# dkogan/horizonator

Hardware: AMD Instinct MI355X
Metric: panorama Mpix/s (360deg, 16k-wide, 7x7 SRTM3 tiles) (higher is better)
Workload: dtype f32

## Files before the change

horizonator_amd/_lib.py:

```python
import ctypes as C
import os

_HERE = os.path.dirname(os.path.abspath(__file__))
LIB_PATH = os.environ.get("HORIZONATOR_AMD_LIB") or os.path.join(_HERE, "libhorizonator.so")
DEMGEN_PATH = os.path.join(_HERE, "libhzdemgen.so")
SELFTEST_PATH = os.path.join(_HERE, "libhorizonator_selftest.so")

MAX_NDEMS_IJ = 4


class DemContext(C.Structure):
    _fields_ = [
        ("dems", (C.c_void_p * MAX_NDEMS_IJ) * MAX_NDEMS_IJ),
        ("mmap_sizes", (C.c_size_t * MAX_NDEMS_IJ) * MAX_NDEMS_IJ),
        ("mmap_fd", (C.c_int * MAX_NDEMS_IJ) * MAX_NDEMS_IJ),
        ("origin_dem_lon_lat", C.c_int * 2),
        ("origin_dem_cellij", C.c_int * 2),
        ("Ndems_ij", C.c_int * 2),
        ("radius_cells", C.c_int),
        ("cells_per_deg", C.c_int),
    ]


class _Offscreen(C.Structure):
# ... 2 lines not shown
        ("frameBufID", C.c_uint32),
        ("renderBufID", C.c_uint32),
        ("depthBufID", C.c_uint32),
        ("width", C.c_int),
        ("height", C.c_int),
    ]


class Context(C.Structure):
    _fields_ = (
        [("Ntriangles", C.c_int), ("render_texture", C.c_bool), ("use_glut", C.c_bool),
         ("glut_window", C.c_int)]
        + [(name, C.c_int32) for name in (
            "uniform_aspect", "uniform_az_deg0", "uniform_az_deg1",
            "uniform_viewer_cell_i", "uniform_viewer_cell_j", "uniform_viewer_z",
            "uniform_viewer_lat", "uniform_cos_viewer_lat",
            "uniform_texturemap_lon0", "uniform_texturemap_lon1",
            "uniform_texturemap_dlat0", "uniform_texturemap_dlat1", "uniform_texturemap_dlat2",
            "uniform_znear", "uniform_zfar", "uniform_znear_color", "uniform_zfar_color")]
        + [("program", C.c_uint32), ("viewer_lat", C.c_float), ("viewer_lon", C.c_float),
           ("dems", DemContext), ("offscreen", _Offscreen)]
    )


class View(C.Structure):
    _fields_ = [(n, C.c_float) for n in (
        "viewer_cell_i", "viewer_cell_j", "viewer_z", "cos_viewer_lat", "deg_per_cell",
        "az_deg0", "az_deg1", "aspect", "znear", "zfar", "znear_color", "zfar_color")]


class Options(C.Structure):
    _fields_ = [(n, C.c_int) for n in (
        "serial", "rounds", "near_cells", "coarse_depth", "tiles", "tile_list", "adapt", "adapt_hi", "pretest_march",
        "worklists", "fast_math", "resolve_clears", "queue_capacity", "host_dense", "host_sectors", "host_times", "vertex_cache")]


class Times(C.Structure):
    _fields_ = [(n, C.c_float) for n in ("clear_ms", "raster_ms", "big_ms", "resolve_ms", "total_ms", "near_ms")]


class Window(C.Structure):
    _fields_ = [("cells_per_deg", C.c_int), ("radius_cells", C.c_int),
                ("origin_tile", C.c_int * 2), ("origin_cell", C.c_int * 2)]


class TexParams(C.Structure):
    _fields_ = [(n, C.c_float) for n in ("viewer_lat_rad", "origin_cell_lon_deg", "origin_cell_lat_deg",
                                         "lon0", "lon1", "dlat0", "dlat1", "dlat2")] + \
               [(n, C.c_int32) for n in ("ntiles_x", "ntiles_y", "lowest_x", "lowest_y", "tex_w", "tex_h")]


RASTER_AUTO, RASTER_SCATTER, RASTER_MARCH = 0, 1, 2

_lib = None
_selftest = None


def load():
    global _lib
    if _lib is None:
        _lib = _open(LIB_PATH, selftest=os.path.basename(LIB_PATH) == os.path.basename(SELFTEST_PATH))
    return _lib


def load_selftest():
    global _selftest
    if _selftest is None:
# ... 79 lines not shown
    sig("hz_hip_set_options", i, vp, P(Options))
    sig("hz_hip_set_texture", i, vp, P(TexParams), vp)
    sig("hz_hip_pack", i, vp, vp)
    sig("hz_hip_resolve_packed", i, vp, P(View), vp, vp, i, i, i, vp, vp)
    sig("hz_hip_pack_sparse", i, vp, vp, i)
    sig("hz_hip_resolve_sparse", i, vp, P(View), vp, vp, i, i, i, vp, vp)
    sig("hz_hip_resolve_sparse_strips", i, vp, P(View), vp, i, vp, i, vp, vp, vp, vp)
    sig("hz_hip_draw", i, vp, P(View))
    sig("hz_hip_resolve", i, vp, P(View), vp, vp, vp, vp, vp)
    sig("hz_hip_resolve_to_host", i, vp, P(View), vp, vp, vp, vp, vp)
    sig("hz_hip_render_to_host", i, vp, P(View), vp, vp, vp, vp, vp)
    sig("hz_hip_host_begin", i, vp, P(View), vp, vp, vp, vp, vp)
    sig("hz_hip_host_end", i, vp)
    sig("hz_hip_host_prepare", i, vp, i, i, i, i, vp)
    sig("hz_hip_read_depth", i, vp, i, i, P(C.c_uint32))
    sig("hz_hip_link_cells", i, vp, P(View), vp, vp, vp, vp, d, d, d, i, i, i, i, vp, vp)
    sig("hz_hip_poi_visibility", i, vp, P(View), vp, i, vp, i, vp, vp, vp)
    sig("hz_hip_sync", i, vp)
    sig("hz_hip_last_times", i, vp, P(Times))
    sig("hz_hip_stream", vp, vp)
    sig("hz_hip_wait_outputs", i, vp, vp)
    sig("hz_hip_wait_for", i, vp, vp)
    sig("horizonator_amd_stream_waits_for_outputs", b, ctxp, vp)
    sig("horizonator_amd_waits_for_stream", b, ctxp, vp)
    sig("hz_hip_last_plan", i, vp, vp)
    sig("hz_hip_last_queue_counts", i, vp, vp)
    sig("hz_hip_last_error", C.c_char_p)
    if selftest:
        sig("hz_hip_check_fastmath", i, i, i, C.c_uint64, C.c_uint64, P(C.c_uint64), vp)
        sig("hz_hip_check_exactness", i, i, i, C.c_uint64, C.c_uint64, i, i, i, i, P(C.c_uint64))
        sig("hz_hip_debug_bigqueue", i, vp, i, vp, i, vp)
        sig("hz_hip_debug_wave_timing", i, vp, P(View), vp, C.c_size_t, vp)
        sig("hz_hip_debug_worklist", C.c_long, i, i, i, P(View), i, i, i, vp, C.c_size_t)
    return lib


DECLARED_SYMBOLS = [
    "horizonator_init", "horizonator_deinit", "horizonator_resized", "horizonator_pan_zoom",
    "horizonator_move", "horizonator_set_zextents", "horizonator_redraw", "horizonator_pick",
    "horizonator_render_offscreen", "horizonator_x_from_az", "horizonator_project",
    "horizonator_unproject",
    "horizonator_dem_init", "horizonator_dem_deinit", "horizonator_dem_sample",
    "horizonator_dem_bounds_latlon_deg",
    "horizonator_amd_get_window", "horizonator_amd_init_from_mosaic",
    "horizonator_amd_render", "horizonator_amd_render_device", "horizonator_amd_render_batch",
    "horizonator_amd_render_packed", "horizonator_amd_resolve_packed",
    "horizonator_amd_resolve_packed_strips", "horizonator_amd_render_sparse",
    "horizonator_amd_resolve_sparse_strips",
    "horizonator_amd_sync", "horizonator_amd_stream_waits_for_outputs", "horizonator_amd_waits_for_stream", "horizonator_amd_texture_layout", "horizonator_amd_set_texture",
    "horizonator_amd_set_sector", "horizonator_amd_set_raster", "horizonator_amd_set_profiling",
    "horizonator_amd_get_options", "horizonator_amd_set_options", "horizonator_amd_render_begin", "horizonator_amd_render_end",
    "horizonator_amd_last_times", "horizonator_amd_get_view", "horizonator_amd_device",
    "horizonator_amd_get_mosaic", "horizonator_amd_link_cells_size", "horizonator_amd_link_cells",
    "horizonator_amd_poi_visibility", "horizonator_amd_build_id",
    "hz_hip_device_count", "hz_hip_create", "hz_hip_destroy", "hz_hip_upload_mosaic",
    "hz_hip_download_mosaic", "hz_hip_ingest_tiles", "hz_hip_set_sector", "hz_hip_set_raster",
    "hz_hip_set_profiling", "hz_hip_get_options", "hz_hip_set_options", "hz_hip_set_texture", "hz_hip_pack", "hz_hip_resolve_packed", "hz_hip_pack_sparse", "hz_hip_resolve_sparse", "hz_hip_resolve_sparse_strips", "hz_hip_draw", "hz_hip_resolve", "hz_hip_resolve_to_host", "hz_hip_render_to_host", "hz_hip_host_begin", "hz_hip_host_end", "hz_hip_host_prepare",
    "hz_hip_read_depth", "hz_hip_link_cells", "hz_hip_poi_visibility", "hz_hip_sync", "hz_hip_last_times", "hz_hip_stream", "hz_hip_wait_outputs", "hz_hip_wait_for", "hz_hip_last_plan", "hz_hip_last_queue_counts", "hz_hip_last_error",
]
SELFTEST_SYMBOLS = ["hz_hip_check_fastmath", "hz_hip_check_exactness", "hz_hip_debug_bigqueue", "hz_hip_debug_wave_timing",
                    "hz_hip_debug_worklist"]


def load_demgen():
    if not os.path.exists(DEMGEN_PATH):
        raise ImportError(f"{DEMGEN_PATH} is missing: build it with `make -C horizonator_amd/csrc`")
    lib = C.CDLL(DEMGEN_PATH)
    lib.hz_demgen_write_region.restype = C.c_int
    lib.hz_demgen_write_region.argtypes = [C.c_char_p] + [C.c_int] * 6
    lib.hz_demgen_write_tile.restype = C.c_int
    lib.hz_demgen_write_tile.argtypes = [C.c_char_p] + [C.c_int] * 4
    lib.hz_demgen_tile_values.restype = None
    lib.hz_demgen_tile_values.argtypes = [C.c_void_p] + [C.c_int] * 4
    return lib
```

horizonator_amd/csrc/hz_context.cpp:

```cpp
#include "hz_dev.h"

#include <time.h>

thread_local char hz_g_last_error[512];
extern "C" const char* hz_hip_last_error(void) { return g_last_error; }


static int env_int(const char* name, int dflt) { const char* e = getenv(name); return e ? atoi(e) : dflt; }
static hz_options_t default_options(void)
{
    hz_options_t o;
    o.serial         = 0;
    o.rounds         = 0;
    o.near_cells     = -1;
    o.coarse_depth   = -1;
    o.tiles          = -1;
    o.tile_list      = 0;
    o.adapt          = 1;
    o.adapt_hi       = -1;
    o.pretest_march  = -1;
    o.worklists      = 1;
    o.fast_math      = 1;
    o.resolve_clears = 1;
    o.queue_capacity = 0;
    o.host_dense     = 0;
    o.host_sectors   = 0;
    o.host_times     = 0;
    o.vertex_cache   = 1;
    return o;
}
hz_options_t hz_options_from_env(void)
{
    hz_options_t o = default_options();
    o.serial         = env_int("HZ_SERIAL", o.serial) != 0;
    if(getenv("HZ_TWO_PASS")) o.rounds = env_int("HZ_TWO_PASS", 0) != 0 ? 2 : 1;
    o.near_cells     = env_int("HZ_NEAR_CELLS", o.near_cells);
    if(getenv("HZ_HIZ")) o.coarse_depth = env_int("HZ_HIZ", 0) != 0;
    o.tiles          = env_int("HZ_TILES", o.tiles);
    o.tile_list      = env_int("HZ_TILE_LIST", o.tile_list);
    o.adapt          = env_int("HZ_ADAPT", o.adapt);
    o.adapt_hi       = env_int("HZ_ADAPT_HI", o.adapt_hi);
    if(getenv("HZ_PRETEST_MARCH")) o.pretest_march = env_int("HZ_PRETEST_MARCH", 0) != 0;
    o.worklists      = env_int("HZ_NO_WORKLIST", 0) == 0;
    o.fast_math      = env_int("HZ_NO_FAST_MATH", 0) == 0;
    o.resolve_clears = env_int("HZ_RESOLVE_CLEARS", o.resolve_clears) != 0;
    o.queue_capacity = env_int("HZ_QUEUE_CAPACITY", o.queue_capacity);
    o.host_dense     = env_int("HZ_HOST_DENSE", o.host_dense) != 0;
    o.host_sectors   = env_int("HZ_HOST_SECTORS", o.host_sectors);
    o.host_times     = env_int("HZ_HOST_TIMES", o.host_times) != 0;
    o.vertex_cache   = env_int("HZ_VERTEX_CACHE", o.vertex_cache) != 0;
    return o;
}
#ifdef HZ_EXPERIMENTS
static hz_experiments_t experiments_from_env(void)
{
    hz_experiments_t e = { env_int("HZ_MARCH_DEBUG", 0), env_int("HZ_EXP_FB_MARCH", 0), env_int("HZ_EXP_FB_BIG", 0) };
    return e;
}
#endif
extern "C" int hz_hip_device_count(void)
{
    int n = 0;
    if(hipGetDeviceCount(&n) != hipSuccess) return 0;
    return n;
}

hipError_t hz_sync_all(hz_dev_t* d)
{
    hipError_t rc = hipSuccess;
    hipStream_t all[4] = { d->stream, d->nstream, d->qstream, d->rstream };
    for(int k=0; k<4; k++)
        if(all[k]) { const hipError_t e = hipStreamSynchronize(all[k]); if(e != hipSuccess) rc = e; }
    return rc;
}

extern "C" void hz_hip_destroy(hz_dev_t* d)
{
    if(!d) return;
    hz_device_guard device_guard_(d->device);
    (void)hz_sync_all(d);
    (void)hipFree(d->d_mosaic);
    for(int i=0; i<HZ_NFB; i++) { (void)hipFree(d->d_fbs[i]); (void)hipFree(d->d_touched[i]); }
    for(int i=0; i<2*HZ_NFB; i++)
// ... 329 lines not shown
```

horizonator_amd/csrc/hz_dev.h:

```cpp
#pragma once

#include <hip/hip_runtime_api.h>

#include <math.h>
#include <stdio.h>
#include <stdlib.h>
#include <string.h>
#include <time.h>

#include <vector>

#include "hz_hip.h"
#include "hz_types.h"
#include "hz_launch.h"


extern thread_local char hz_g_last_error[512];
#define g_last_error hz_g_last_error

#define HZ_CHECK(call)                                                        \
    do {                                                                      \
        hipError_t e_ = (call);                                               \
        if(e_ != hipSuccess)                                                  \
        {                                                                     \
// ... 2 lines not shown
            fprintf(stderr, "hz_hip: %s\n", g_last_error);                    \
            return -1;                                                        \
        }                                                                     \
    } while(0)

struct hz_device_guard
{
    int prev, dev; bool ok;
    explicit hz_device_guard(int device) : prev(-1), dev(device), ok(true)
    {
        if(hipGetDevice(&prev) != hipSuccess) prev = -1;
        if(prev != dev)
        {
            const hipError_t e = hipSetDevice(dev);
            if(e != hipSuccess)
            {
                ok = false;
                snprintf(g_last_error, sizeof(g_last_error), "hipSetDevice(%d) -> %s", dev, hipGetErrorString(e));
                fprintf(stderr, "hz_hip: %s\n", g_last_error);
            }
        }
    }
    ~hz_device_guard() { if(ok && prev >= 0 && prev != dev) (void)hipSetDevice(prev); }
};
#define HZ_ON_DEVICE(d) hz_device_guard device_guard_((d)->device); if(!device_guard_.ok) return -1

#ifdef HZ_EXPERIMENTS
struct hz_experiments_t { int march_debug, exp_fb_march, exp_fb_big; };
#endif

struct hz_listkey_t
{
    hz_view_t view; int col0, col1, two_pass, near_x0, near_x1, near_j0, near_j1, far_rows;
};
#define HZ_NLISTS 2
struct hz_worklists_t
{
    uint32_t*    d_items[HZ_NLISTS];
    uint32_t*    h_items[HZ_NLISTS][2];
    size_t       cap[HZ_NLISTS];
    unsigned int n[HZ_NLISTS];
    hipEvent_t   ev_copied[HZ_NLISTS][2];
    int          turn[HZ_NLISTS];
    int          valid;
    unsigned int last_used;
    hz_listkey_t key;
};
#define HZ_LIST_CACHE 8

struct hz_dev
{
    int device;
    hz_options_t env;
#ifdef HZ_EXPERIMENTS
    hz_experiments_t exp;
#endif
    int N, W, H;
    int col0, col1;
    int raster;
    int profiling;
    hz_worklists_t list_cache[HZ_LIST_CACHE];
    hz_worklists_t* lists;
    unsigned int lists_clock;
    std::vector<uint32_t>* list_scratch;
    std::vector<uint32_t>* list_scratch2;
    struct { unsigned long long* d_cycles; size_t capacity; unsigned int grid_x, grid_y; } wave_timing;
// ... 53 lines not shown

    hipEvent_t ev[10];
    int        have_times;
    hz_times_t times;
};

#define HZ_NEAR_PX            20.0f
#define HZ_TWO_ROUNDS_MIN_PIX 6.0e6
#define HZ_TILES_MIN_PX       35.0f
#define HZ_HIZ_MIN_PX         25.0f



struct hz_stopwatch
{
    bool on; timespec t0;
    explicit hz_stopwatch(const char* var) : on(getenv(var) && atoi(getenv(var)) != 0) { clock_gettime(CLOCK_MONOTONIC, &t0); }
    void lap(const char* what)
    {
        if(!on) return;
        timespec t1; clock_gettime(CLOCK_MONOTONIC, &t1);
        fprintf(stderr, "hz_hip init: %-34s %8.2f ms\n", what, 1e3*(double)(t1.tv_sec - t0.tv_sec) + 1e-6*(double)(t1.tv_nsec - t0.tv_nsec));
        t0 = t1;
    }
};


hz_options_t hz_options_from_env(void);
mr_queue_t   hz_queue_set(const hz_dev_t* d, int k);
int          hz_tile_bins(hz_dev_t* d, int set);
hipError_t   hz_sync_all(hz_dev_t* d);
hz_params_t  hz_make_params(const hz_dev_t* d, const hz_view_t* v);
int          hz_plan_rounds(const hz_dev_t* d, const hz_view_t* view, hz_params_t& p);
mr_zones_t   hz_make_zones(const hz_params_t& p, bool near_first);
bool         hz_azimuths_of_columns(const hz_params_t& p, double* a0, double* a1);
void         hz_list_items(const hz_params_t& p, const mr_zones_t& zn, double a0, double a1, std::vector<uint32_t>& out, bool every_strip = false);
void         hz_list_rounds(const hz_params_t& p, const mr_zones_t& zn, double a0, double a1, bool one_round,
                            std::vector<uint32_t>* first, std::vector<uint32_t>& second, bool every_strip = false);
int          hz_draw_impl(hz_dev_t* d, const hz_view_t* view);
int          hz_fb_refill(hz_dev_t* d);
int          hz_fb_mark_consumed(hz_dev_t* d);
int          hz_upload_tanel(hz_dev_t* d, const float* tanel);
int          hz_rstream_after_draw(hz_dev_t* d);
int          hz_resolve_impl(hz_dev_t* d, const hz_view_t* view, const float* tanel,
                             unsigned char* bgr, float* ranges, int32_t* index, uint32_t* z24, int nbands, hipEvent_t* ev_band, int* band_rows);
void         hz_hostpath_destroy(hz_dev_t* d);
int          hz_gpu_numa_node(const hz_dev_t* d);
void         hz_hostpath_landing(hz_dev_t* d, unsigned char** pinned, size_t* bytes);
```

horizonator_amd/csrc/hz_draw.cpp:

```cpp
#include "hz_dev.h"
#include "hz_fast.h"

static int upload_list(hz_dev_t* d, int which, hipStream_t st, const std::vector<uint32_t>& items)
{
    hz_worklists_t& wl = *d->lists;
    const size_t n = items.size();
    if(n > wl.cap[which])
    {
        HZ_CHECK(hz_sync_all(d));
        (void)hipFree(wl.d_items[which]); wl.d_items[which] = NULL;
        for(int t=0; t<2; t++) { if(wl.h_items[which][t]) (void)hipHostFree(wl.h_items[which][t]); wl.h_items[which][t] = NULL; }
        wl.cap[which] = 0;
        const size_t cap = n + n/4 + 1024;
        hipError_t e = hipMalloc(&wl.d_items[which], cap*sizeof(uint32_t));
        for(int t=0; t<2 && e == hipSuccess; t++) e = hipHostMalloc((void**)&wl.h_items[which][t], cap*sizeof(uint32_t), hipHostMallocDefault);
        if(e != hipSuccess)
        {
            (void)hipFree(wl.d_items[which]); wl.d_items[which] = NULL;
            for(int t=0; t<2; t++) { if(wl.h_items[which][t]) (void)hipHostFree(wl.h_items[which][t]); wl.h_items[which][t] = NULL; }
            HZ_CHECK(e);
        }
        wl.cap[which] = cap;
    }
    const int t = wl.turn[which]; wl.turn[which] ^= 1;
// ... 192 lines not shown
                d->adapt.items_short = items;
                const double hi = d->env.adapt_hi >= 0 ? (double)d->env.adapt_hi : 500000.0*((double)(d->col1 - d->col0)*(double)d->H/64.0e6);
                if(!d->adapt.tried_long && (double)items > hi) d->adapt.long_reach = 1;
            }
            else
            {
                d->adapt.tried_long = 1;
                if(!(d->adapt.items_short && (unsigned long long)items*10ull < (unsigned long long)d->adapt.items_short*7ull)) d->adapt.long_reach = 0;
            }
        }
    (void)hipGetLastError();
    if(next_framebuffer(d, p) != 0) return -1;
    const int next = d->fbi;
    if(d->raster != HZ_RASTER_SCATTER && vertex_cache(d, p) != 0) return -1;

    const mr_queue_t q = hz_queue_set(d, next);
    bool by_tile_first = d->env.tiles > 0 && d->raster != HZ_RASTER_SCATTER;
    bool near_beside_far = false;
    bool waited_near = false;
    bool use_hiz = false;
    bool zoomed_view = false;

    if(d->raster == HZ_RASTER_SCATTER)
    {
        HZ_CHECK(hipStreamWaitEvent(d->stream, d->ev_free[next], 0));
        if(prof) { HZ_CHECK(hipEventRecord(d->ev[7], d->stream)); HZ_CHECK(hipEventRecord(d->ev[6], d->stream)); HZ_CHECK(hipEventRecord(d->ev[9], d->stream)); }
        dim3 grid((p.N-1 + SC_CX-1)/SC_CX, (p.N-1 + SC_CY-1)/SC_CY);
        hzk_scatter(grid, dim3(SC_THREADS), d->stream, (const int16_t*)d->d_mosaic, d->d_fb, q, p);
        HZ_CHECK(hipGetLastError());
    }
    else
    {
        const bool two_pass = hz_plan_rounds(d, view, p) == 2;
        const mr_zones_t zn = hz_make_zones(p, two_pass);
        double a0 = 0, a1 = 0;
        const bool listed = d->env.worklists && hz_azimuths_of_columns(p, &a0, &a1) && zn.total < (1 << (32 - MR_ITEM_SX_BITS))
                            && (p.N-1 + MR_COLS-1)/MR_COLS <= (1 << MR_ITEM_SX_BITS);
        p.cull_strips = (p.col0 > 0 || p.col1 < p.W || listed) ? 1 : 0;
        bool fresh_lists = false;
        if(listed)
        {
            hz_listkey_t key;
            memset(&key, 0, sizeof(key));
            key.view = *view; key.col0 = p.col0; key.col1 = p.col1; key.two_pass = two_pass ? 1 : 0;
            key.near_x0 = p.near_x0; key.near_x1 = p.near_x1; key.near_j0 = p.near_j0; key.near_j1 = p.near_j1; key.far_rows = zn.rows[0] | (zn.rows[1] << 8);
            hz_worklists_t* hit = NULL; hz_worklists_t* lru = &d->list_cache[0];
            for(int c=0; c<HZ_LIST_CACHE; c++)
            {
                hz_worklists_t* e = &d->list_cache[c];
                if(e->valid && memcmp(&key, &e->key, sizeof(key)) == 0) { hit = e; break; }
                if((!e->valid && lru->valid) || (e->valid == lru->valid && e->last_used < lru->last_used)) lru = e;
            }
            fresh_lists = hit == NULL;
            d->lists = hit ? hit : lru;
            d->lists->last_used = ++d->lists_clock;
            if(fresh_lists) { d->lists->valid = 0; d->lists->key = key; }
        }
        if(two_pass)
        {
            p.inline_max = HZ_INLINE_MAX_PIX;
            const mr_queue_t qn = hz_queue_set(d, HZ_NFB + next);
            HZ_CHECK(hipStreamWaitEvent(d->nstream, d->ev_free[next], 0));
            {
                const float ppr = p.halfW * p.u.az_ndc_per_rad;
                const float reach = 0.5f*(float)(p.near_j1 - p.near_j0);
                zoomed_view = reach > 0.f && ppr/reach >= HZ_HIZ_MIN_PX;
                const float cells_to_zfar = view->zfar / (p.u.deg_per_cell * 111194.9f);
                p.qshards_log2 = (zoomed_view || cells_to_zfar <= 0.25f*ppr) ? HZ_QSHARDS_LOG2 : 0;
            }
            hz_params_t p1 = p;
            p1.pass = 1; p1.early_z = 0;
            if(fresh_lists)
            {
                hz_list_rounds(p1, zn, a0, a1, false, d->list_scratch, *d->list_scratch2);
                if(upload_list(d, 0, d->nstream, *d->list_scratch) != 0) return -1;
            }
            if(prof) HZ_CHECK(hipEventRecord(d->ev[7], d->nstream));
            if(launch_march(d, d->nstream, qn, zn, p1, listed ? d->lists->d_items[0] : NULL, d->lists->n[0]) != 0) return -1;
// ... 93 lines not shown
```

horizonator_amd/csrc/hz_k_march.h:

```cpp
#pragma once


#define MR_CAP    128
#define MR_RSLOTS 4
#define MR_FIELDS 6

struct mr_lds_t
{
    uint32_t rows[MR_RSLOTS][MR_FIELDS][64];
    uint32_t ids[MR_CAP];
    uint32_t clip[64];
    uint32_t nclip;
};

__device__ static inline void mr_clip_flush(mr_lds_t& L, const mr_queue_t& q, int lane)
{
    const unsigned int nclip = (unsigned int)__builtin_amdgcn_readfirstlane((int)L.nclip);
    if(!nclip) return;
    uint32_t base = 0;
    if(lane == 0) base = atomicAdd(&q.counters[4], nclip);
    base = (uint32_t)__builtin_amdgcn_readfirstlane((int)base);
    if((unsigned int)lane < nclip)
    {
        const uint32_t at = base + (uint32_t)lane;
// ... 376 lines not shown
    }
    if(dbg) { const uint32_t tot = (uint32_t)__builtin_amdgcn_readlane((int)mr_scan(npix, lane), 63); dbg[4] += tot; }
    mr_distribute(r, npix, lane, fb, p);
}

#ifdef MR_WAVES_PER_EU
#define MR_OCCUPANCY __attribute__((amdgpu_waves_per_eu(MR_WAVES_PER_EU, MR_WAVES_PER_EU)))
#elif defined(MR_VGPRS)
#define MR_OCCUPANCY __attribute__((amdgpu_num_vgpr(MR_VGPRS)))
#else
#define MR_OCCUPANCY
#endif
template<bool COUNTERS, bool HIZ, bool VCACHE, bool SHARDS>
__global__ __launch_bounds__(64) MR_OCCUPANCY
void k_march(const int16_t* __restrict__ mosaic, unsigned long long* __restrict__ fb,
             mr_queue_t q, mr_zones_t zn, hz_params_t p)
{
    __shared__ mr_lds_t L;
    const unsigned long long t_start = COUNTERS ? __builtin_amdgcn_s_memtime() : 0ull;
    unsigned int dbgv[6] = {0,0,0,0,0,0};
    unsigned int* dbg = COUNTERS ? dbgv : nullptr;

    const int lane = threadIdx.x;
    int sx, seg;
    if(p.worklist)
    {
        const uint32_t item = p.worklist[blockIdx.x];
        sx = (int)(item & ((1u << MR_ITEM_SX_BITS) - 1u)); seg = (int)(item >> MR_ITEM_SX_BITS);
    }
    else { sx = (int)blockIdx.x + (p.pass == 1 ? p.near_x0 : 0); seg = (int)blockIdx.y; }
    const int i0   = sx*MR_COLS;
    const int i    = i0 + lane;
    int jbeg, jend;
    mr_segment_rows(zn, seg, &jbeg, &jend);
    if(p.pass)
    {
        const bool near = sx >= p.near_x0 && sx <= p.near_x1 && jbeg < p.near_j1 && jend > p.near_j0;
        if((p.pass == 1) != near) return;
    }
    const bool has_vertex = i < p.N;
    const bool has_cell   = lane < MR_COLS && i < p.N-1;
    const int  ic = has_vertex ? i : p.N-1;

    if(p.cull_strips)
    {
        const int ia = i0, ib = min(i0 + MR_COLS, p.N-1);
        const bool viewer_inside = p.u.viewer_cell_i >= (float)(ia-1) && p.u.viewer_cell_i <= (float)(ib+1) &&
                                   p.u.viewer_cell_j >= (float)(jbeg-1) && p.u.viewer_cell_j <= (float)(jend+1);
        if(!viewer_inside)
        {
            const hz_vertex_t v = hz_transform_en(&p.u, hz_east(&p.u, (float)((lane & 1) ? ib : ia)),
                                                  hz_north(&p.u, (float)((lane & 2) ? jend : jbeg)), 0.f);
            float xlo = 2.f, xhi = -2.f;
            #pragma unroll
            for(int c=0; c<4; c++)
            {
                const float xc = __builtin_bit_cast(float, __builtin_amdgcn_readlane(__builtin_bit_cast(int, v.x), c));
                xlo = hz_min(xlo, xc); xhi = hz_max(xhi, xc);
            }
            if(xhi - xlo <= 1.0f)
            {
                const float flo = (xlo*p.halfW + p.halfW) - 2.5f, fhi = (xhi*p.halfW + p.halfW) + 1.5f;
                if(fhi < (float)p.col0 || flo > (float)p.col1) return;
            }
        }
    }

// ... 162 lines not shown
```

horizonator_amd/csrc/hz_plan.cpp:

```cpp
#include "hz_dev.h"
#include "hz_fast.h"

mr_zones_t hz_make_zones(const hz_params_t& p, bool near_first)
{
    const float ppr = p.halfW * p.u.az_ndc_per_rad;
    const int   ncr = p.N-1;
    const float vj  = p.u.viewer_cell_j;
    const int r2  = (int)(ppr/16.f) + 1;
    const int r4  = (int)(ppr/4.f) + 1;
    const int r16 = (int)(ppr/1.f) + 1;
    auto clampi = [&](float x) { int v = (int)floorf(x); if(v < 0) v = 0; if(v > ncr) v = ncr; return v; };
    mr_zones_t z;
    z.row0[0] = 0;
    z.row0[1] = clampi(vj - (float)r16);
    z.row0[2] = clampi(vj - (float)r4);
    z.row0[3] = clampi(vj - (float)r2);
    z.row0[4] = clampi(vj + (float)r2 + 1.f);
    z.row0[5] = clampi(vj + (float)r4 + 1.f);
    z.row0[6] = clampi(vj + (float)r16 + 1.f);
    z.row0[7] = ncr;
    int far_rows = 64*p.SW/p.W;
    if(far_rows < 16) far_rows = 16;
    if(far_rows > 32) far_rows = 32;
    const int z16 = 6*p.SW < p.W ? 8 : 16;
    const float cells_to_zfar = sqrtf(p.far_dd)/(p.u.deg_per_cell*111194.9f);
    const int z4 = cells_to_zfar <= 0.25f*ppr ? 2 : 4;
    int rows[MR_NZONES] = { far_rows, z16, z4, 2, z4, z16, far_rows };
    if(p.SW == p.W)
    {
        long waves = 0;
        for(int k=0; k<MR_NZONES; k++) waves += (z.row0[k+1] - z.row0[k] + rows[k]-1)/rows[k];
        waves *= (p.N-1 + MR_COLS-1)/MR_COLS;
        if(waves < 32768) { rows[0] = rows[6] = rows[0] < 16 ? rows[0] : 16; rows[1] = rows[5] = rows[1] < 8 ? rows[1] : 8; rows[2] = rows[4] = 2; }
    }
    const int order_far_first [MR_NZONES] = { 0, 6, 1, 5, 2, 4, 3 };
    const int order_near_first[MR_NZONES] = { 3, 2, 4, 1, 5, 0, 6 };
    z.near_first = near_first ? 1 : 0;
    const int* order = near_first ? order_near_first : order_far_first;
    int seg = 0;
    for(int o=0; o<MR_NZONES; o++)
    {
        const int k = order[o];
        z.rows[k] = rows[k];
        z.seg0[k] = seg;
        const int n = z.row0[k+1] - z.row0[k];
        z.nseg[k] = (n + rows[k]-1)/rows[k];
        seg += z.nseg[k];
    }
    z.total = seg;
    return z;
}

hz_params_t hz_make_params(const hz_dev_t* d, const hz_view_t* v)
{
    hz_params_t p;
    memset(&p, 0, sizeof(p));
    p.u.viewer_cell_i  = v->viewer_cell_i;
    p.u.viewer_cell_j  = v->viewer_cell_j;
    p.u.viewer_z       = v->viewer_z;
    p.u.cos_viewer_lat = v->cos_viewer_lat;
    p.u.deg_per_cell   = v->deg_per_cell;
    p.u.aspect         = v->aspect;
    p.u.znear          = v->znear;
    p.u.zfar           = v->zfar;
    p.u.znear_color    = v->znear_color;
    p.u.zfar_color     = v->zfar_color;
// ... 85 lines not shown
    }
    if(!any) return false;
    double i_lo = lo/m_per_cell_e + (double)p.u.viewer_cell_i - 2.0, i_hi = hi/m_per_cell_e + (double)p.u.viewer_cell_i + 2.0;
    if(!(i_lo > -1e9)) i_lo = -1e9;
    if(!(i_hi <  1e9)) i_hi =  1e9;
    int a = (int)ceil(i_lo/(double)MR_COLS) - 1, b = (int)floor(i_hi/(double)MR_COLS);
    if(a < 0) a = 0;
    if(b > nsx-1) b = nsx-1;
    if(a > b) return false;
    *x0 = a; *x1 = b;
    return true;
}

bool hz_azimuths_of_columns(const hz_params_t& p, double* a0, double* a1)
{
    const double k = (double)p.u.az_ndc_per_rad, c = (double)p.u.az_center, hw = (double)p.halfW;
    const double lo = c + (((double)p.col0 - 4.0)/hw - 1.0)/k, hi = c + (((double)p.col1 + 4.0)/hw - 1.0)/k;
    if(!(hi - lo < 2.0*M_PI - 1e-3) || !(hi > lo)) return false;
    *a0 = lo; *a1 = hi;
    return true;
}

void hz_list_rounds(const hz_params_t& p, const mr_zones_t& zn, double a0, double a1, bool one_round,
                    std::vector<uint32_t>* first, std::vector<uint32_t>& second, bool every_strip)
{
    const int nsx = (p.N-1 + MR_COLS-1)/MR_COLS;
    if(first) first->clear();
    second.clear();
    const double m_per_cell_n = (double)HZ_REARTH_PI * (double)p.u.deg_per_cell / 180.0;
    const double m_per_cell_e = m_per_cell_n * (double)p.u.cos_viewer_lat;
    const int parts = (a1 - a0 > M_PI) ? 2 : 1;
    double ray[3][2];
    for(int k=0; k<=parts; k++) { const double a = a0 + (a1 - a0)*k/parts; ray[k][0] = sin(a); ray[k][1] = cos(a); }
    for(int seg=0; seg<zn.total; seg++)
    {
        int jbeg, jend;
        mr_segment_rows(zn, seg, &jbeg, &jend);
        int x0 = 0, x1 = nsx-1;
        if(!every_strip && !strips_behind_columns(p, a0, a1, jbeg, jend, nsx, &x0, &x1)) continue;
        const bool near_rows = jbeg < p.near_j1 && jend > p.near_j0;
        const double n_lo = ((double)(jbeg-1) - (double)p.u.viewer_cell_j) * m_per_cell_n;
        const double n_hi = ((double)(jend+1) - (double)p.u.viewer_cell_j) * m_per_cell_n;
        auto reaches = [&](int sx) -> bool
        {
            const double e_lo = ((double)(sx*MR_COLS - 2) - (double)p.u.viewer_cell_i) * m_per_cell_e;
            const double e_hi = ((double)(sx*MR_COLS + MR_COLS + 2) - (double)p.u.viewer_cell_i) * m_per_cell_e;
            if(e_lo <= 0.0 && 0.0 <= e_hi && n_lo <= 0.0 && 0.0 <= n_hi) return true;
            for(int k=0; k<parts; k++)
            {
                const double c[4][2] = { { e_lo, n_lo }, { e_hi, n_lo }, { e_lo, n_hi }, { e_hi, n_hi } };
                bool before_first = true, beyond_second = true;
                for(int q=0; q<4; q++)
                {
                    if(!(ray[k][0]*c[q][1] - ray[k][1]*c[q][0] > 0.0))   before_first = false;
                    if(!(ray[k+1][0]*c[q][1] - ray[k+1][1]*c[q][0] < 0.0)) beyond_second = false;
                }
                if(!before_first && !beyond_second) return true;
            }
            return false;
        };
        if(!every_strip && parts == 1)
        {
            while(x0 <= x1 && !reaches(x0)) x0++;
            while(x1 > x0 && !reaches(x1)) x1--;
        }
        for(int sx=x0; sx<=x1; sx++)
        {
            if(!every_strip && parts == 2 && !reaches(sx)) continue;
            const bool near = !one_round && near_rows && sx >= p.near_x0 && sx <= p.near_x1;
            if(near) { if(first) first->push_back(MR_ITEM(seg, sx)); }
            else second.push_back(MR_ITEM(seg, sx));
        }
    }
}

void hz_list_items(const hz_params_t& p, const mr_zones_t& zn, double a0, double a1, std::vector<uint32_t>& out, bool every_strip)
{
    if(p.pass == 1) { std::vector<uint32_t> rest; hz_list_rounds(p, zn, a0, a1, false, &out, rest, every_strip); }
    else hz_list_rounds(p, zn, a0, a1, p.pass == 0, NULL, out, every_strip);
}

int hz_plan_rounds(const hz_dev_t* d, const hz_view_t* view, hz_params_t& p)
{
    const int nsx = (p.N-1 + MR_COLS-1)/MR_COLS;
    int near_cells = d->env.near_cells;
    if(near_cells < 0)
    {
        const float ppr = p.halfW * p.u.az_ndc_per_rad;
        near_cells = (int)(ppr / HZ_NEAR_PX + 0.5f);
        if(near_cells < 16) near_cells = 16;
        if(near_cells > HZ_NEAR_CELLS_WIDE) near_cells = HZ_NEAR_CELLS_WIDE;
        if(ppr/(float)HZ_NEAR_CELLS_MAX >= HZ_HIZ_MIN_PX && (d->env.adapt == 2 || (d->env.adapt == 1 && d->adapt.long_reach))) near_cells = HZ_NEAR_CELLS_MAX;
    }
    p.near_x0 = (int)floorf((p.u.viewer_cell_i - (float)near_cells)/(float)MR_COLS);
    p.near_x1 = (int)floorf((p.u.viewer_cell_i + (float)near_cells)/(float)MR_COLS);
    if(p.near_x0 < 0) p.near_x0 = 0;
    if(p.near_x1 > nsx-1) p.near_x1 = nsx-1;
    p.near_j0 = (int)floorf(p.u.viewer_cell_j - (float)near_cells);
    p.near_j1 = (int)ceilf (p.u.viewer_cell_j + (float)near_cells);
    const float cells_to_zfar = view->zfar / (p.u.deg_per_cell * 111194.9f);
    const bool want_two = d->env.rounds > 0 ? d->env.rounds == 2
                             : ((double)p.W*(double)p.H >= HZ_TWO_ROUNDS_MIN_PIX && cells_to_zfar >= 3.0f*(float)near_cells);
    return want_two && near_cells > 0 && p.near_x1 >= p.near_x0 ? 2 : 1;
}
```

horizonator_amd/csrc/hz_selftest_impl.h:

```cpp
#pragma once

__device__ static inline unsigned long long hz_mix64(unsigned long long x)
{
    x += 0x9E3779B97F4A7C15ull;
    x = (x ^ (x >> 30)) * 0xBF58476D1CE4E5B9ull;
    x = (x ^ (x >> 27)) * 0x94D049BB133111EBull;
    return x ^ (x >> 31);
}
__device__ static inline float hz_seeded_float(unsigned long long r, int elo, int ehi)
{
    const uint32_t mant = (uint32_t)r & 0x7FFFFFu, sign = (uint32_t)(r >> 23) & 1u;
    const uint32_t ex = (uint32_t)elo + (uint32_t)((r >> 24) % (unsigned long long)(ehi - elo + 1));
    return __uint_as_float((sign << 31) | (ex << 23) | mant);
}

__global__ __launch_bounds__(256)
void k_check_fastmath(int what, unsigned long long seed, unsigned long long n, unsigned long long* mismatches, float* first_bad)
{
    unsigned long long bad = 0;
    for(unsigned long long k = (unsigned long long)blockIdx.x*blockDim.x + threadIdx.x; k < n; k += (unsigned long long)gridDim.x*blockDim.x)
    {
        float a = 0.f, b = 0.f, want = 0.f, got = 0.f;
        bool in_range = true;
        if(what == 0)
// ... 349 lines not shown
        }
        counters[4] = all[4];
    }
    counters[2] = ~counters[2]; counters[5] = ~counters[5];
    if(longest == 0 || recs == NULL || max_rec <= 0) return 0;
    const size_t slots = (size_t)((longest + HZ_QBLOCK-1)/HZ_QBLOCK*HZ_QBLOCK) << sl;
    hz_bigrec_t* h = (hz_bigrec_t*)malloc(slots*sizeof(hz_bigrec_t));
    if(!h) return -1;
    HZ_CHECK(hipMemcpy(h, d->d_bigrec_s[k], slots*sizeof(hz_bigrec_t), hipMemcpyDeviceToHost));
    int n = 0;
    for(size_t g=0; g<slots && n<max_rec; g++)
    {
        const size_t block = g >> HZ_QBLOCK_LOG2;
        if((((block >> sl) << HZ_QBLOCK_LOG2) | (g & (HZ_QBLOCK-1))) >= per_shard[block & (((size_t)1 << sl) - 1)]) continue;
        int32_t* o = recs + (size_t)n*10;
        o[0] = h[g].r.px0; o[1] = h[g].r.py0; o[2] = h[g].r.bw; o[3] = h[g].bh;
        for(int m=0; m<3; m++) { o[4+m] = h[g].r.e.dx[m]; o[7+m] = -h[g].r.e.ndy[m]; }
        n++;
    }
    free(h);
    return 0;
}

extern "C" long hz_hip_debug_worklist(int N, int W, int H, const hz_view_t* view, int col0, int col1, int round,
                                      int32_t* out, size_t capacity_items)
{
    hz_dev_t* d = (hz_dev_t*)calloc(1, sizeof(*d));
    if(!d) return -1;
    d->env = hz_options_from_env();
    d->N = N; d->W = W; d->H = H; d->col0 = col0; d->col1 = col1;
    d->seg_stride = (W + HZ_SEG-1)/HZ_SEG;
    hz_params_t p = hz_make_params(d, view);
    (void)hz_plan_rounds(d, view, p);
    const mr_zones_t zn = hz_make_zones(p, (round & 3) != 0);
    free(d);
    p.pass = round & 3;
    double a0 = 0, a1 = 0;
    const bool every_strip = (round & 256) != 0;
    if(!every_strip && !hz_azimuths_of_columns(p, &a0, &a1)) return -1;
    std::vector<uint32_t> items;
    hz_list_items(p, zn, a0, a1, items, every_strip);
    for(size_t k=0; k<items.size() && k<capacity_items; k++)
    {
        int jbeg, jend;
        mr_segment_rows(zn, (int)(items[k] >> MR_ITEM_SX_BITS), &jbeg, &jend);
        out[3*k] = (int32_t)(items[k] & ((1u << MR_ITEM_SX_BITS) - 1u)); out[3*k+1] = jbeg; out[3*k+2] = jend;
    }
    return (long)items.size();
}

extern "C" int hz_hip_debug_wave_timing(hz_dev_t* d, const hz_view_t* view, unsigned long long* out, size_t capacity_words, unsigned int* grid)
{
    HZ_ON_DEVICE(d);
    HZ_CHECK(hz_sync_all(d));
    unsigned long long* d_cycles = NULL;
    HZ_CHECK(hipMalloc(&d_cycles, capacity_words*sizeof(unsigned long long)));
    HZ_CHECK(hipMemset(d_cycles, 0, capacity_words*sizeof(unsigned long long)));
    d->wave_timing.d_cycles = d_cycles; d->wave_timing.capacity = capacity_words;
    d->wave_timing.grid_x = d->wave_timing.grid_y = 0;
    int rc = hz_draw_impl(d, view);
    d->wave_timing.d_cycles = NULL; d->wave_timing.capacity = 0;
    if(rc == 0 && hz_sync_all(d) != hipSuccess) rc = -1;
    grid[0] = d->wave_timing.grid_x; grid[1] = d->wave_timing.grid_y;
    if(rc == 0 && hipMemcpy(out, d_cycles, (size_t)grid[0]*grid[1]*4*sizeof(unsigned long long), hipMemcpyDeviceToHost) != hipSuccess) rc = -1;
    (void)hipFree(d_cycles);
    return rc;
}
```

horizonator_amd/csrc/hz_types.h:

```cpp
#pragma once

#include <stddef.h>
#include <stdint.h>

#include "hz_raster.h"
#include "hz_tex.h"
#include "hz_scatter.h"


struct hz_hiz_t { uint32_t* l1; uint32_t* l2; int w1, w2; };

#define HZ_WHO_MARCH 0
#define HZ_WHO_BIG   1
#define HZ_WHO_OTHER 2

struct hz_params_t
{
    hz_xform_t u;
    float halfW, halfH;
    int   N;
    int   W, H;
    int   col0, col1;
    int   SW;
    unsigned long long* wave_cycles;
// ... 52 lines not shown
#define HZ_QSHARDS_LOG2  4
#define HZ_QSHARDS       (1 << HZ_QSHARDS_LOG2)
#define HZ_QBLOCK_LOG2   4
#define HZ_QBLOCK        (1 << HZ_QBLOCK_LOG2)
#define HZ_QSHARD_ROOM(capacity, sl) ((((capacity) >> ((sl) + HZ_QBLOCK_LOG2))) << HZ_QBLOCK_LOG2)
#define HZ_QSLOT(l, s, sl) (((((((uint32_t)(l)) >> HZ_QBLOCK_LOG2) << (sl)) + (uint32_t)(s)) << HZ_QBLOCK_LOG2) | (((uint32_t)(l)) & (HZ_QBLOCK-1)))
#define HZ_QSHARD_STRIDE 32
#define HZ_QSHARD0       16
#define HZ_NCOUNTERS (HZ_QSHARD0 + HZ_QSHARDS*HZ_QSHARD_STRIDE)
#define HZ_CNT_LAST  8
#ifndef HZ_NFB
#define HZ_NFB 3
#endif
#define HZ_STAGE_SLOTS 32
#define HZ_STAGE_BYTES ((size_t)4 << 20)
#define HZ_COPY_STREAMS 2
#define HZ_HOST_BANDS  4
#define HZ_INLINE_MAX_PIX  64


#define MR_COLS   63
#define HZ_NEAR_CELLS_WIDE 384
#define HZ_NEAR_CELLS_MAX  512

#define MR_NZONES 7
struct mr_zones_t
{
    int row0[MR_NZONES+1];
    int rows[MR_NZONES];
    int seg0[MR_NZONES];
    int nseg[MR_NZONES];
    int total;
    int near_first;
};

HZ_HD void mr_segment_rows(const mr_zones_t& zn, int seg, int* jbeg, int* jend)
{
    int zone = 0;
    #pragma unroll
    for(int z=1; z<MR_NZONES; z++)
        if(seg >= zn.seg0[z] && seg < zn.seg0[z] + zn.nseg[z]) zone = z;
    int sseg = seg - zn.seg0[zone];
    if(zn.near_first && zone < MR_NZONES/2) sseg = zn.nseg[zone]-1 - sseg;
    const int jb = zn.row0[zone] + sseg*zn.rows[zone];
    const int je = jb + zn.rows[zone];
    *jbeg = jb;
    *jend = je < zn.row0[zone+1] ? je : zn.row0[zone+1];
}

#define MR_ITEM_SX_BITS 12
#define MR_ITEM(seg, sx) (((uint32_t)(seg) << MR_ITEM_SX_BITS) | (uint32_t)(sx))


#define TL_W 64
#define TL_H 64

#define TL_LIST 2048
#define TL_BATCH 64
#define TL_ROW_MIN 24
#define TL_UNITS_PER_TILE 4

struct tl_bins_t
{
    unsigned int* cursor;
    unsigned int* pairs;
    unsigned int* state;
    unsigned int* busy;
    unsigned int  units_cap;
    int           tiles_x, tiles_y;
    unsigned int  list_cap;
};

#define HIZ1_W_LOG2 3
#define HIZ1_H_LOG2 2
#define HIZ2_W_LOG2 5
#define HIZ2_H_LOG2 4
#define HIZ_UNIT_ROWS 16

HZ_HD size_t hiz_w1(int SW) { return (size_t)((SW + (1 << HIZ1_W_LOG2) - 1) >> HIZ1_W_LOG2); }
HZ_HD size_t hiz_w2(int SW) { return (size_t)((SW + (1 << HIZ2_W_LOG2) - 1) >> HIZ2_W_LOG2); }
// ... 47 lines not shown
```

include/hz_hip.h:

```cpp
#pragma once

#include <stddef.h>
#include <stdint.h>

#ifdef __cplusplus
extern "C" {
#endif

typedef struct hz_dev hz_dev_t;

typedef struct
{
    float viewer_cell_i, viewer_cell_j;
    float viewer_z;
    float cos_viewer_lat;
    float deg_per_cell;
    float az_deg0, az_deg1;
    float aspect;
    float znear, zfar;
    float znear_color, zfar_color;
} hz_view_t;

enum
{
// ... 21 lines not shown

int  hz_hip_ingest_tiles(hz_dev_t* d,
                         const unsigned char* const* tiles,
                         int ntiles_lon, int ntiles_lat,
                         int cells_per_deg,
                         int origin_cell_lon, int origin_cell_lat);

int  hz_hip_download_mosaic(hz_dev_t* d, int16_t* mosaic);

int  hz_hip_set_sector(hz_dev_t* d, int col0, int col1);

int  hz_hip_set_raster(hz_dev_t* d, int which);
int  hz_hip_set_profiling(hz_dev_t* d, int on);

typedef struct
{
    int serial;
    int rounds;
    int near_cells;
    int coarse_depth;
    int tiles;
    int tile_list;
    int adapt;
    int adapt_hi;
    int pretest_march;
    int worklists;
    int fast_math;
    int resolve_clears;
    int queue_capacity;
    int host_dense;
    int host_sectors;
    int host_times;
    int vertex_cache;
} hz_options_t;
int  hz_hip_get_options(hz_dev_t* d, hz_options_t* o);
int  hz_hip_set_options(hz_dev_t* d, const hz_options_t* o);

int  hz_hip_draw(hz_dev_t* d, const hz_view_t* view);

int  hz_hip_resolve(hz_dev_t* d, const hz_view_t* view, const float* tanel,
                    unsigned char* bgr, float* ranges, int32_t* index, uint32_t* z24);

int  hz_hip_resolve_to_host(hz_dev_t* d, const hz_view_t* view, const float* tanel,
                            unsigned char* bgr, float* ranges, int32_t* index, uint32_t* z24);
int  hz_hip_render_to_host(hz_dev_t* d, const hz_view_t* view, const float* tanel,
                           unsigned char* bgr, float* ranges, int32_t* index, uint32_t* z24);
int  hz_hip_host_begin(hz_dev_t* d, const hz_view_t* view, const float* tanel,
                       unsigned char* bgr, float* ranges, int32_t* index, uint32_t* z24);
int  hz_hip_host_end(hz_dev_t* d);
int  hz_hip_host_prepare(hz_dev_t* d, int want_bgr, int want_ranges, int want_index, int want_z24, const hz_view_t* warm_view);

int  hz_hip_read_depth(hz_dev_t* d, int x, int y, uint32_t* z24);


int  hz_hip_link_cells(hz_dev_t* d, const hz_view_t* view, const float* tanel,
                       const float* sin_az, const float* cos_az, const double* cos_el,
                       double viewer_lat, double cos_viewer_lat, double viewer_lon,
                       int cell_w, int cell_h, int nx, int ny, float* lat, float* lon);

typedef struct { float lat, lon, ele_m; } hz_poi_t;
typedef struct { double x, y, range; } hz_poi_proj_t;

int  hz_hip_poi_visibility(hz_dev_t* d, const hz_view_t* view, const float* tanel,
                           int cut_off_bottom_px, const hz_poi_proj_t* proj, int npois,
                           unsigned char* visible, float* label_x, float* label_y);

// ... 40 lines not shown
```

include/hz_selftest.h:

```cpp
#pragma once

#include "hz_hip.h"

#ifdef __cplusplus
extern "C" {
#endif

int  hz_hip_check_fastmath(int device, int what, unsigned long long seed, unsigned long long n,
                           unsigned long long* mismatches, float* first_bad);

int  hz_hip_check_exactness(int device, int what, unsigned long long seed, unsigned long long n,
                            int W, int H, int col0, int col1, unsigned long long* out);

int  hz_hip_debug_bigqueue(hz_dev_t* d, int set, unsigned int* counters, int max_rec, int32_t* recs);

long hz_hip_debug_worklist(int N, int W, int H, const hz_view_t* view, int col0, int col1, int round,
                           int32_t* out, size_t capacity_items);

int  hz_hip_debug_wave_timing(hz_dev_t* d, const hz_view_t* view, unsigned long long* out, size_t capacity_words, unsigned int* grid);

#ifdef __cplusplus
}
#endif
```

Measured before the change: 84920.

## Merge mid-zone row segments into taller work items for strips far from viewer

Adds a far_merge option, on by default, that finds a column-strip window around the viewer. Outside that window, the mid zones (2-4) of the march kernel get a per-zone shift that widens each segment's row span up to 16 rows. The aim is fewer, larger work items for distant strips, cutting per-wave launch and setup overhead. The cost is fewer parallel items and more empty segment slots, which the kernel and the worklist builder now skip. Segment-row lookup takes the strip index, the worklist cache key includes the new shift parameters, and a debug entry point is added.

```diff
diff --git a/horizonator_amd/_lib.py b/horizonator_amd/_lib.py
--- a/horizonator_amd/_lib.py
+++ b/horizonator_amd/_lib.py
@@ -58,7 +58,7 @@
 class Options(C.Structure):
     _fields_ = [(n, C.c_int) for n in (
         "serial", "rounds", "near_cells", "coarse_depth", "tiles", "tile_list", "adapt", "adapt_hi", "pretest_march",
-        "worklists", "fast_math", "resolve_clears", "queue_capacity", "host_dense", "host_sectors", "host_times", "vertex_cache")]
+        "worklists", "fast_math", "resolve_clears", "queue_capacity", "host_dense", "host_sectors", "host_times", "vertex_cache", "far_merge")]
 
 
 class Times(C.Structure):
@@ -204,6 +204,7 @@
         sig("hz_hip_debug_bigqueue", i, vp, i, vp, i, vp)
         sig("hz_hip_debug_wave_timing", i, vp, P(View), vp, C.c_size_t, vp)
         sig("hz_hip_debug_worklist", C.c_long, i, i, i, P(View), i, i, i, vp, C.c_size_t)
+        sig("hz_hip_debug_segment_rows", i, i, i, i, P(View), i, i, i, i, i, vp)
     return lib
 
 
@@ -231,7 +232,7 @@
     "hz_hip_read_depth", "hz_hip_link_cells", "hz_hip_poi_visibility", "hz_hip_sync", "hz_hip_last_times", "hz_hip_stream", "hz_hip_wait_outputs", "hz_hip_wait_for", "hz_hip_last_plan", "hz_hip_last_queue_counts", "hz_hip_last_error",
 ]
 SELFTEST_SYMBOLS = ["hz_hip_check_fastmath", "hz_hip_check_exactness", "hz_hip_debug_bigqueue", "hz_hip_debug_wave_timing",
-                    "hz_hip_debug_worklist"]
+                    "hz_hip_debug_worklist", "hz_hip_debug_segment_rows"]
 
 
 def load_demgen():
diff --git a/horizonator_amd/csrc/hz_context.cpp b/horizonator_amd/csrc/hz_context.cpp
--- a/horizonator_amd/csrc/hz_context.cpp
+++ b/horizonator_amd/csrc/hz_context.cpp
@@ -27,6 +27,7 @@
     o.host_sectors   = 0;
     o.host_times     = 0;
     o.vertex_cache   = 1;
+    o.far_merge      = 1;
     return o;
 }
 hz_options_t hz_options_from_env(void)
@@ -49,6 +50,7 @@
     o.host_sectors   = env_int("HZ_HOST_SECTORS", o.host_sectors);
     o.host_times     = env_int("HZ_HOST_TIMES", o.host_times) != 0;
     o.vertex_cache   = env_int("HZ_VERTEX_CACHE", o.vertex_cache) != 0;
+    o.far_merge      = env_int("HZ_FAR_MERGE", o.far_merge) != 0;
     return o;
 }
 #ifdef HZ_EXPERIMENTS
diff --git a/horizonator_amd/csrc/hz_dev.h b/horizonator_amd/csrc/hz_dev.h
--- a/horizonator_amd/csrc/hz_dev.h
+++ b/horizonator_amd/csrc/hz_dev.h
@@ -58,6 +58,7 @@
 struct hz_listkey_t
 {
     hz_view_t view; int col0, col1, two_pass, near_x0, near_x1, near_j0, near_j1, far_rows;
+    int far_shifts, far_sx0, far_sx1;
 };
 #define HZ_NLISTS 2
 struct hz_worklists_t
@@ -177,7 +178,7 @@
 hipError_t   hz_sync_all(hz_dev_t* d);
 hz_params_t  hz_make_params(const hz_dev_t* d, const hz_view_t* v);
 int          hz_plan_rounds(const hz_dev_t* d, const hz_view_t* view, hz_params_t& p);
-mr_zones_t   hz_make_zones(const hz_params_t& p, bool near_first);
+mr_zones_t   hz_make_zones(const hz_params_t& p, bool near_first, bool far_merge);
 bool         hz_azimuths_of_columns(const hz_params_t& p, double* a0, double* a1);
 void         hz_list_items(const hz_params_t& p, const mr_zones_t& zn, double a0, double a1, std::vector<uint32_t>& out, bool every_strip = false);
 void         hz_list_rounds(const hz_params_t& p, const mr_zones_t& zn, double a0, double a1, bool one_round,
diff --git a/horizonator_amd/csrc/hz_draw.cpp b/horizonator_amd/csrc/hz_draw.cpp
--- a/horizonator_amd/csrc/hz_draw.cpp
+++ b/horizonator_amd/csrc/hz_draw.cpp
@@ -248,7 +248,7 @@
     else
     {
         const bool two_pass = hz_plan_rounds(d, view, p) == 2;
-        const mr_zones_t zn = hz_make_zones(p, two_pass);
+        const mr_zones_t zn = hz_make_zones(p, two_pass, d->env.far_merge != 0);
         double a0 = 0, a1 = 0;
         const bool listed = d->env.worklists && hz_azimuths_of_columns(p, &a0, &a1) && zn.total < (1 << (32 - MR_ITEM_SX_BITS))
                             && (p.N-1 + MR_COLS-1)/MR_COLS <= (1 << MR_ITEM_SX_BITS);
@@ -260,6 +260,7 @@
             memset(&key, 0, sizeof(key));
             key.view = *view; key.col0 = p.col0; key.col1 = p.col1; key.two_pass = two_pass ? 1 : 0;
             key.near_x0 = p.near_x0; key.near_x1 = p.near_x1; key.near_j0 = p.near_j0; key.near_j1 = p.near_j1; key.far_rows = zn.rows[0] | (zn.rows[1] << 8);
+            key.far_shifts = zn.shift[2] | (zn.shift[3] << 8) | (zn.shift[4] << 16); key.far_sx0 = zn.near_sx0; key.far_sx1 = zn.near_sx1;
             hz_worklists_t* hit = NULL; hz_worklists_t* lru = &d->list_cache[0];
             for(int c=0; c<HZ_LIST_CACHE; c++)
             {
diff --git a/horizonator_amd/csrc/hz_k_march.h b/horizonator_amd/csrc/hz_k_march.h
--- a/horizonator_amd/csrc/hz_k_march.h
+++ b/horizonator_amd/csrc/hz_k_march.h
@@ -432,7 +432,8 @@
     const int i0   = sx*MR_COLS;
     const int i    = i0 + lane;
     int jbeg, jend;
-    mr_segment_rows(zn, seg, &jbeg, &jend);
+    mr_segment_rows(zn, sx, seg, &jbeg, &jend);
+    if(jbeg >= jend) return;
     if(p.pass)
     {
         const bool near = sx >= p.near_x0 && sx <= p.near_x1 && jbeg < p.near_j1 && jend > p.near_j0;
diff --git a/horizonator_amd/csrc/hz_plan.cpp b/horizonator_amd/csrc/hz_plan.cpp
--- a/horizonator_amd/csrc/hz_plan.cpp
+++ b/horizonator_amd/csrc/hz_plan.cpp
@@ -1,10 +1,11 @@
 #include "hz_dev.h"
 #include "hz_fast.h"
 
-mr_zones_t hz_make_zones(const hz_params_t& p, bool near_first)
+mr_zones_t hz_make_zones(const hz_params_t& p, bool near_first, bool far_merge)
 {
     const float ppr = p.halfW * p.u.az_ndc_per_rad;
     const int   ncr = p.N-1;
+    const int   nsx = (p.N-1 + MR_COLS-1)/MR_COLS;
     const float vj  = p.u.viewer_cell_j;
     const int r2  = (int)(ppr/16.f) + 1;
     const int r4  = (int)(ppr/4.f) + 1;
@@ -26,12 +27,46 @@
     const float cells_to_zfar = sqrtf(p.far_dd)/(p.u.deg_per_cell*111194.9f);
     const int z4 = cells_to_zfar <= 0.25f*ppr ? 2 : 4;
     int rows[MR_NZONES] = { far_rows, z16, z4, 2, z4, z16, far_rows };
+    z.near_sx0 = 0; z.near_sx1 = nsx-1;
+    const bool merging = far_merge && p.SW == p.W && z4 == 4;
+    if(merging)
+    {
+        const float cosl = p.u.cos_viewer_lat > 1e-6f ? p.u.cos_viewer_lat : 1e-6f;
+        const float reach = (float)r4 / cosl;
+        float lo = floorf((p.u.viewer_cell_i - reach)/(float)MR_COLS) - 1.f, hi = floorf((p.u.viewer_cell_i + reach)/(float)MR_COLS) + 1.f;
+        if(!(lo > 0.f)) lo = 0.f;
+        if(!(lo < (float)nsx)) lo = (float)nsx;
+        if(!(hi > -1.f)) hi = -1.f;
+        if(!(hi < (float)(nsx-1))) hi = (float)(nsx-1);
+        z.near_sx0 = (int)lo; z.near_sx1 = (int)hi;
+        if(z.near_sx0 > z.near_sx1) { z.near_sx0 = 0; z.near_sx1 = nsx-1; }
+        if(p.near_x1 >= p.near_x0)
+        {
+            if(p.near_x0 < z.near_sx0) z.near_sx0 = p.near_x0 < 0 ? 0 : p.near_x0;
+            if(p.near_x1 > z.near_sx1) z.near_sx1 = p.near_x1 > nsx-1 ? nsx-1 : p.near_x1;
+        }
+    }
+    const int far_sx = merging ? z.near_sx0 + (nsx-1 - z.near_sx1) : 0;
+    auto set_shifts = [&]()
+    {
+        const int target = rows[1] < 16 ? rows[1] : 16;
+        for(int k=0; k<MR_NZONES; k++)
+        {
+            z.shift[k] = 0;
+            if(far_sx > 0 && k >= 2 && k <= 4) while((rows[k] << (z.shift[k]+1)) <= target) z.shift[k]++;
+        }
+    };
+    set_shifts();
     if(p.SW == p.W)
     {
         long waves = 0;
-        for(int k=0; k<MR_NZONES; k++) waves += (z.row0[k+1] - z.row0[k] + rows[k]-1)/rows[k];
-        waves *= (p.N-1 + MR_COLS-1)/MR_COLS;
+        for(int k=0; k<MR_NZONES; k++)
+        {
+            const long n = (z.row0[k+1] - z.row0[k] + rows[k]-1)/rows[k];
+            waves += n*(nsx - far_sx) + ((n + (1 << z.shift[k]) - 1) >> z.shift[k])*far_sx;
+        }
         if(waves < 32768) { rows[0] = rows[6] = rows[0] < 16 ? rows[0] : 16; rows[1] = rows[5] = rows[1] < 8 ? rows[1] : 8; rows[2] = rows[4] = 2; }
+        set_shifts();
     }
     const int order_far_first [MR_NZONES] = { 0, 6, 1, 5, 2, 4, 3 };
     const int order_near_first[MR_NZONES] = { 3, 2, 4, 1, 5, 0, 6 };
@@ -183,12 +218,16 @@
     const int parts = (a1 - a0 > M_PI) ? 2 : 1;
     double ray[3][2];
     for(int k=0; k<=parts; k++) { const double a = a0 + (a1 - a0)*k/parts; ray[k][0] = sin(a); ray[k][1] = cos(a); }
-    for(int seg=0; seg<zn.total; seg++)
+    auto list_segment = [&](int seg, int sx_lo, int sx_hi)
     {
         int jbeg, jend;
-        mr_segment_rows(zn, seg, &jbeg, &jend);
+        mr_segment_rows(zn, sx_lo, seg, &jbeg, &jend);
+        if(jbeg >= jend) return;
         int x0 = 0, x1 = nsx-1;
-        if(!every_strip && !strips_behind_columns(p, a0, a1, jbeg, jend, nsx, &x0, &x1)) continue;
+        if(!every_strip && !strips_behind_columns(p, a0, a1, jbeg, jend, nsx, &x0, &x1)) return;
+        if(x0 < sx_lo) x0 = sx_lo;
+        if(x1 > sx_hi) x1 = sx_hi;
+        if(x0 > x1) return;
         const bool near_rows = jbeg < p.near_j1 && jend > p.near_j0;
         const double n_lo = ((double)(jbeg-1) - (double)p.u.viewer_cell_j) * m_per_cell_n;
         const double n_hi = ((double)(jend+1) - (double)p.u.viewer_cell_j) * m_per_cell_n;
@@ -222,6 +261,16 @@
             if(near) { if(first) first->push_back(MR_ITEM(seg, sx)); }
             else second.push_back(MR_ITEM(seg, sx));
         }
+    };
+    bool merged = false;
+    for(int k=0; k<MR_NZONES; k++) if(zn.shift[k]) merged = true;
+    if(zn.near_sx0 <= 0 && zn.near_sx1 >= nsx-1) merged = false;
+    for(int seg=0; seg<zn.total; seg++)
+    {
+        if(!merged) { list_segment(seg, 0, nsx-1); continue; }
+        if(zn.near_sx0 > 0) list_segment(seg, 0, zn.near_sx0-1);
+        list_segment(seg, zn.near_sx0 > 0 ? zn.near_sx0 : 0, zn.near_sx1 < nsx-1 ? zn.near_sx1 : nsx-1);
+        if(zn.near_sx1 < nsx-1) list_segment(seg, zn.near_sx1+1, nsx-1);
     }
 }
 
diff --git a/horizonator_amd/csrc/hz_selftest_impl.h b/horizonator_amd/csrc/hz_selftest_impl.h
--- a/horizonator_amd/csrc/hz_selftest_impl.h
+++ b/horizonator_amd/csrc/hz_selftest_impl.h
@@ -405,7 +405,7 @@
     d->seg_stride = (W + HZ_SEG-1)/HZ_SEG;
     hz_params_t p = hz_make_params(d, view);
     (void)hz_plan_rounds(d, view, p);
-    const mr_zones_t zn = hz_make_zones(p, (round & 3) != 0);
+    const mr_zones_t zn = hz_make_zones(p, (round & 3) != 0, d->env.far_merge != 0);
     free(d);
     p.pass = round & 3;
     double a0 = 0, a1 = 0;
@@ -416,10 +416,37 @@
     for(size_t k=0; k<items.size() && k<capacity_items; k++)
     {
         int jbeg, jend;
-        mr_segment_rows(zn, (int)(items[k] >> MR_ITEM_SX_BITS), &jbeg, &jend);
-        out[3*k] = (int32_t)(items[k] & ((1u << MR_ITEM_SX_BITS) - 1u)); out[3*k+1] = jbeg; out[3*k+2] = jend;
+        const int sx = (int)(items[k] & ((1u << MR_ITEM_SX_BITS) - 1u));
+        mr_segment_rows(zn, sx, (int)(items[k] >> MR_ITEM_SX_BITS), &jbeg, &jend);
+        out[3*k] = (int32_t)sx; out[3*k+1] = jbeg; out[3*k+2] = jend;
     }
     return (long)items.size();
+}
+
+extern "C" int hz_hip_debug_segment_rows(int N, int W, int H, const hz_view_t* view, int col0, int col1, int flags, int sx, int seg, int32_t* out)
+{
+    hz_dev_t* d = (hz_dev_t*)calloc(1, sizeof(*d));
+    if(!d) return -1;
+    d->env = hz_options_from_env();
+    if(flags & 1) d->env.far_merge = 0;
+    if(flags & 2) d->env.rounds = 2;
+    if(flags & 4) d->env.rounds = 1;
+    d->N = N; d->W = W; d->H = H; d->col0 = col0; d->col1 = col1;
+    d->seg_stride = (W + HZ_SEG-1)/HZ_SEG;
+    hz_params_t p = hz_make_params(d, view);
+    const int rounds = hz_plan_rounds(d, view, p);
+    const mr_zones_t zn = hz_make_zones(p, rounds == 2, d->env.far_merge != 0);
+    free(d);
+    const int nsx = (N-1 + MR_COLS-1)/MR_COLS;
+    out[0] = out[1] = 0;
+    out[2] = zn.total; out[3] = nsx; out[4] = p.near_x0; out[5] = p.near_x1; out[6] = p.near_j0; out[7] = p.near_j1;
+    out[8] = zn.near_sx0; out[9] = zn.near_sx1; out[10] = rounds; out[11] = 0;
+    for(int k=0; k<MR_NZONES; k++) if(zn.shift[k] > out[11]) out[11] = zn.shift[k];
+    if(sx < 0 || sx >= nsx || seg < 0 || seg >= zn.total) return 1;
+    int jbeg, jend;
+    mr_segment_rows(zn, sx, seg, &jbeg, &jend);
+    out[0] = jbeg; out[1] = jend;
+    return 0;
 }
 
 extern "C" int hz_hip_debug_wave_timing(hz_dev_t* d, const hz_view_t* view, unsigned long long* out, size_t capacity_words, unsigned int* grid)
diff --git a/horizonator_amd/csrc/hz_types.h b/horizonator_amd/csrc/hz_types.h
--- a/horizonator_amd/csrc/hz_types.h
+++ b/horizonator_amd/csrc/hz_types.h
@@ -108,20 +108,26 @@
     int nseg[MR_NZONES];
     int total;
     int near_first;
-};
-
-HZ_HD void mr_segment_rows(const mr_zones_t& zn, int seg, int* jbeg, int* jend)
+    int shift[MR_NZONES];
+    int near_sx0, near_sx1;
+};
+
+HZ_HD void mr_segment_rows(const mr_zones_t& zn, int sx, int seg, int* jbeg, int* jend)
 {
     int zone = 0;
     #pragma unroll
     for(int z=1; z<MR_NZONES; z++)
         if(seg >= zn.seg0[z] && seg < zn.seg0[z] + zn.nseg[z]) zone = z;
     int sseg = seg - zn.seg0[zone];
-    if(zn.near_first && zone < MR_NZONES/2) sseg = zn.nseg[zone]-1 - sseg;
-    const int jb = zn.row0[zone] + sseg*zn.rows[zone];
-    const int je = jb + zn.rows[zone];
-    *jbeg = jb;
-    *jend = je < zn.row0[zone+1] ? je : zn.row0[zone+1];
+    const int k    = (sx < zn.near_sx0 || sx > zn.near_sx1) ? zn.shift[zone] : 0;
+    const int nseg = (zn.nseg[zone] + (1 << k) - 1) >> k;
+    const int rows = zn.rows[zone] << k;
+    const bool empty = sseg >= nseg;
+    if(zn.near_first && zone < MR_NZONES/2) sseg = nseg-1 - sseg;
+    const int jb = zn.row0[zone] + sseg*rows;
+    const int je = jb + rows;
+    *jbeg = empty ? zn.row0[zone+1] : jb;
+    *jend = (empty || je > zn.row0[zone+1]) ? zn.row0[zone+1] : je;
 }
 
 #define MR_ITEM_SX_BITS 12
diff --git a/include/hz_hip.h b/include/hz_hip.h
--- a/include/hz_hip.h
+++ b/include/hz_hip.h
@@ -77,6 +77,7 @@
     int host_sectors;
     int host_times;
     int vertex_cache;
+    int far_merge;
 } hz_options_t;
 int  hz_hip_get_options(hz_dev_t* d, hz_options_t* o);
 int  hz_hip_set_options(hz_dev_t* d, const hz_options_t* o);
diff --git a/include/hz_selftest.h b/include/hz_selftest.h
--- a/include/hz_selftest.h
+++ b/include/hz_selftest.h
@@ -17,6 +17,8 @@
 long hz_hip_debug_worklist(int N, int W, int H, const hz_view_t* view, int col0, int col1, int round,
                            int32_t* out, size_t capacity_items);
 
+int  hz_hip_debug_segment_rows(int N, int W, int H, const hz_view_t* view, int col0, int col1, int flags, int sx, int seg, int32_t* out);
+
 int  hz_hip_debug_wave_timing(hz_dev_t* d, const hz_view_t* view, unsigned long long* out, size_t capacity_words, unsigned int* grid);
 
 #ifdef __cplusplus
```

Result: no change. 84260 (-0.8%).
